# GmxMahdi/compute-raytracer

Measured on AMD Instinct MI355X. Metric: Mrays/s at 3840x2160, 1024 spheres, 8 bounces, higher is better.
Workload: dtype f32; 1 GPU; C3: 3840x2160, 1024 spheres (seed 358), 8 bounces, constant sky, reference default camera/light; mode=fast, variant=0, rays_per_frame=46143642, frames_in_flight=4, parallelism=row-tiles x1

## Files before the change

### compute_raytracer_amd/csrc/rt_bvh.hip

```cpp
#include <algorithm>
#include <cmath>
#include <cstdlib>
#include <vector>

#include "rt_filter.h"

#define RT_BVH_KAPPA 6.103515625e-05f
#define RT_BVH_REV_DELTA 0.0051f
#define RT_BVH_REV_DELTA_REL 7.62939453125e-06f
#define RT_BVH_REV_SLACK 2.44140625e-04f
#define RT_BVH_REV_SLACK_ABS 4.76837158203125e-07f

#ifndef RT_BVH_GRAB
#define RT_BVH_GRAB 256u
#endif
#ifndef RT_BVH_TAIL_SMALL
#define RT_BVH_TAIL_SMALL 16
#endif
#ifndef RT_BVH_TAIL_SERIAL
#define RT_BVH_TAIL_SERIAL 12
#endif
#ifndef RT_BVH_TAIL_LARGE
#define RT_BVH_TAIL_LARGE 28
#endif

namespace rtk {

__host__ __device__ inline uint32_t bvh_lds_l0(uint32_t n_nodes, uint32_t base) {
    uint32_t l0 = 1024u;
    const uint32_t need = (4u * (n_nodes + 1u) + 2u) / 3u;
    if (base + l0 < need) l0 = need - base;
    return (l0 + 15u) & ~15u;
}
__host__ __device__ inline uint32_t bvh_gap_waves(uint32_t n_nodes, uint32_t waves) {
    const uint32_t k = (bvh_lds_l0(n_nodes, 0u) - 1024u) / 512u;
    return k < waves ? k : waves;
}
__host__ __device__ constexpr uint32_t bvh_list_bytes(bool nlds, uint32_t cap) { return nlds ? 128u * (cap + 1u) : 256u * cap; }
__host__ __device__ inline uint32_t bvh_lds_lists(uint32_t n_nodes, uint32_t base) {
    const uint32_t l0 = bvh_lds_l0(n_nodes, base);
    return 4u * (base + l0) - base + 16u * ((n_nodes + 4u) & ~3u);
}

__global__ void bvh_fill_leaves(float4* rec, const uint32_t* link, uint32_t n_nodes, const float4* geo_f) {
    const uint32_t i = blockIdx.x * blockDim.x + threadIdx.x;
    if (i >= n_nodes) return;
    const uint32_t l = link[i];
    if (l & 0x80000000u) rec[i] = geo_f[l & 0x7FFFFFFFu];
}

__device__ __forceinline__ double wave_max_f64(double v) {
#pragma unroll
    for (int off = 32; off > 0; off >>= 1) v = fmax(v, __shfl_xor(v, off, 64));
    return v;
}
__device__ __forceinline__ double wave_min_f64(double v) {
#pragma unroll
    for (int off = 32; off > 0; off >>= 1) v = fmin(v, __shfl_xor(v, off, 64));
    return v;
}

__global__ __launch_bounds__(256) void bvh_refit(float4* __restrict__ rec, const uint32_t* __restrict__ link,
                                                  uint32_t n_nodes, const float* __restrict__ records) {
    const uint32_t node = blockIdx.x * 4u + (threadIdx.x >> 6), lane = threadIdx.x & 63u;
    if (node >= n_nodes) return;
    const uint32_t lk = link[node];
    if (lk & 0x80000000u) return;
    const uint32_t first = node + 1u, end = lk >> 2;
    auto sphere = [&](uint32_t j, double c[3], double& r) -> bool {
        if (j >= end) return false;
        const uint32_t l = link[j];
        if (!(l & 0x80000000u)) return false;
        const float* s = records + 8u * (size_t)(l & 0x7FFFFFFFu);
        for (int a = 0; a < 3; ++a) { const double v = (double)s[a]; c[a] = v == v ? v : 0.0; }
        const double rv = fabs((double)s[7]);
        r = rv == rv ? rv : 0.0;
        return true;
    };
    auto radius_at = [&](const double P[3], double far[3]) -> double {
        double best = -1.0, bc[3] = {0.0, 0.0, 0.0};
        for (uint32_t j = first + lane; j < end; j += 64u) {
            double c[3], r;
            if (!sphere(j, c, r)) continue;
            const double dx = c[0] - P[0], dy = c[1] - P[1], dz = c[2] - P[2];
            const double d = sqrt(dx * dx + dy * dy + dz * dz) + r;
            if (d > best) { best = d; bc[0] = c[0]; bc[1] = c[1]; bc[2] = c[2]; }
        }
        const double R = wave_max_f64(best);
        const uint64_t who = __ballot(best == R);
        const int src = who ? (int)__builtin_ctzll(who) : 0;
        for (int a = 0; a < 3; ++a) far[a] = __shfl(bc[a], src, 64);
        return R;
    };
    double mn[3] = {INFINITY, INFINITY, INFINITY}, mx[3] = {-INFINITY, -INFINITY, -INFINITY};
    for (uint32_t j = first + lane; j < end; j += 64u) {
        double c[3], r;
        if (!sphere(j, c, r)) continue;
        for (int a = 0; a < 3; ++a) { mn[a] = fmin(mn[a], c[a] - r); mx[a] = fmax(mx[a], c[a] + r); }
    }
    double P[3];
    for (int a = 0; a < 3; ++a) P[a] = 0.5 * (wave_min_f64(mn[a]) + wave_max_f64(mx[a]));
    double far[3];
    double Rp = radius_at(P, far);
    for (int it = 0; it < 32; ++it) {
        const double sx = far[0] - P[0], sy = far[1] - P[1], sz = far[2] - P[2];
        const double len = sqrt(sx * sx + sy * sy + sz * sz);
        if (!(len > 1e-12)) break;
        const double Q[3] = {P[0] + sx / len * 0.05 * Rp, P[1] + sy / len * 0.05 * Rp, P[2] + sz / len * 0.05 * Rp};
        double farq[3];
        const double Rq = radius_at(Q, farq);
        if (!(Rq < Rp)) break;
        P[0] = Q[0]; P[1] = Q[1]; P[2] = Q[2]; Rp = Rq;
        far[0] = farq[0]; far[1] = farq[1]; far[2] = farq[2];
    }
    const float C[3] = {(float)P[0], (float)P[1], (float)P[2]};
    const double Cd[3] = {(double)C[0], (double)C[1], (double)C[2]};
    double unused[3];
    double R = radius_at(Cd, unused);
    R *= RT_BVH_SIGMA;
    const double c2 = Cd[0] * Cd[0] + Cd[1] * Cd[1] + Cd[2] * Cd[2];
    const double k = c2 * (1.0 - (double)RT_FILTER_EPS) - R * R * (1.0 + (double)RT_FILTER_KAPPA);
    if (lane == 0)
        rec[node] = make_float4(C[0] * RT_FILTER_SCALE, C[1] * RT_FILTER_SCALE, C[2] * RT_FILTER_SCALE,
                                (float)(k * (double)RT_FILTER_SCALE2));
}

#ifdef RT_BVH_COUNT
#define g_steps steps_acc
__device__ unsigned long long g_wave_clock[3 * 8192];
#endif
__device__ __forceinline__ float min0(float b) {
    float d; asm("v_min_f32 %0, 0, %1" : "=v"(d) : "v"(b)); return d;
}

__device__ __forceinline__ void exact_any_order(v3 center, float r2, int s, v3 o, v3 d, float fa, float ta,
                                                float& nearest, int& idx) {
    const v3 oc = sub(o, center);
    const float b = 2.0f * dot(d, oc);
    const float c = dot(oc, oc) - r2;
    const float disc = b * b - fa * c;
    if (disc > 0.0f && b < 0.0f) {
        const float t = (-b - sqrtf(disc)) / ta;
        if (t > 0.001f && (t < nearest || (t == nearest && idx >= 0 && s < idx))) {
            nearest = t;
            idx = s;
        }
    }
}

__device__ __forceinline__ void reversed_shadow_walk(bool shadow, v3 L, float light_l1, v3 P, v3 s, v3& wo, v3& wd, float& madd) {
    const v3 dl = sub(P, L);
    const float l1 = (__builtin_fabsf(dl.x) + __builtin_fabsf(dl.y)) + __builtin_fabsf(dl.z);
    const float la = l1 + light_l1;
    const float delta = __builtin_fmaf(la, RT_BVH_REV_DELTA_REL, RT_BVH_REV_DELTA);
    const float lb = l1 + delta;
    const float slack = __builtin_fmaf(lb * lb, RT_BVH_REV_SLACK, (la * la) * RT_BVH_REV_SLACK_ABS);
    if (shadow) {
        wo = V(__builtin_fmaf(delta, s.x, P.x), __builtin_fmaf(delta, s.y, P.y), __builtin_fmaf(delta, s.z, P.z));
        wd = V(-s.x, -s.y, -s.z);
        madd = slack;
    }
}

template <bool SGN, bool NLDS, int CAP, bool ROOMY>
__device__ __forceinline__ void trace_bvh(const uint32_t tail, const float4* __restrict__ R, const uint32_t* __restrict__ L, uint32_t n,
                                          const float4* __restrict__ geo, uint32_t* slot, unsigned long long* best,
                                          uint32_t& i, v3 o, v3 d, v3 wo, v3 wd, float madd, float& nearest, int& idx
#ifdef RT_BVH_COUNT
                                          , uint32_t& steps_acc
#endif
                                          ) {
    const float a = dot(wd, wd);
    const float inv = __builtin_amdgcn_rsqf(a) * (1.0f + RT_BVH_KAPPA);
    const v3 h = V(wd.x * inv, wd.y * inv, wd.z * inv);
    const v3 os = V(wo.x * RT_FILTER_SCALE, wo.y * RT_FILTER_SCALE, wo.z * RT_FILTER_SCALE);
    const v3 m = V(-2.0f * os.x, -2.0f * os.y, -2.0f * os.z);
    const float p = dot(h, os);
    const float q = __builtin_fmaf(-madd, RT_FILTER_SCALE2, dot(os, os) * (1.0f - RT_FILTER_EPS));
    constexpr bool CLAMPED = SGN && NLDS;
    constexpr float kT = 2.168404344971009e-19f;
    constexpr float kT2 = 4.70197740328915e-38f;
    const v3 hs = V(h.x * kT, h.y * kT, h.z * kT);
    const v3 ms = V(m.x * kT2, m.y * kT2, m.z * kT2);
    const float ps = -p * kT, qs = q * kT2;
    typedef __attribute__((address_space(3))) uint32_t* lds_u32_w;
    typedef __attribute__((address_space(3))) uint16_t* lds_u16_w;
    const uint32_t wa0 = (uint32_t)(uintptr_t)slot;
    uint32_t wa = wa0;

    constexpr bool L16 = NLDS;
    typedef __attribute__((address_space(3))) const uint16_t* lds_u16;
    typedef __attribute__((address_space(3))) const uint32_t* lds_u32r;
    auto drain = [&]() {
        const uint32_t lane = threadIdx.x & 63u;
        const uint32_t cnt = L16 ? (wa - wa0) >> 7 : (wa - wa0) >> 8;
        uint32_t* const pool = slot - lane;
        const uint32_t top = wa0 - 2u * lane + 128u * (uint32_t)(CAP + 1);
        uint32_t total = 0;
        uint32_t lim = cnt;
        uint32_t again = 0;
        best[lane] = ((unsigned long long)__float_as_uint(nearest) << 32) | (unsigned long long)(uint32_t)idx;
      for (;;) {
        if (L16) {
            total = 0;
            uint32_t kstop = 0;
            bool stopped = false;
#pragma unroll
            for (int k = CAP - 1; k >= 0; --k) {
                const uint64_t m = __ballot((uint32_t)k < lim);
                if (m == 0ull) continue;
                const uint32_t need = (uint32_t)__popcll(m);
                if (!stopped && 4u * (total + need) > 128u * (uint32_t)(CAP + 1 - k)) { stopped = true; kstop = (uint32_t)k + 1u; }
                if (stopped) continue;
                uint32_t e = 0;
                if ((uint32_t)k < lim) e = *(lds_u16)(uintptr_t)(wa0 + 128u * (uint32_t)k);
                const uint32_t pos = total + __builtin_amdgcn_mbcnt_hi((uint32_t)(m >> 32), __builtin_amdgcn_mbcnt_lo((uint32_t)m, 0u));
                if ((uint32_t)k < lim) *(lds_u32_w)(uintptr_t)(top - 4u - 4u * pos) = (lane << 24) | e;
                total += need;
                asm volatile("" : "+s"(total));
            }
            again = stopped ? 1u : 0u;
            if (stopped) lim = lim < kstop ? lim : kstop;
        } else {
        for (uint32_t k = 0;; ++k) {
            const uint64_t m = __ballot(k < cnt);
            if (m == 0ull) break;
            uint32_t e = 0;
            if (k < cnt) e = slot[k * 64u];
            const uint32_t pos = total + (uint32_t)__popcll(m & ((1ull << lane) - 1ull));
            if (k < cnt) pool[pos] = (lane << 24) | (e & 0x00FFFFFFu);
            total += (uint32_t)__popcll(m);
        }
        }
        for (uint32_t i = lane; __ballot(i < total) != 0ull; i += 64u) {
#ifdef RT_BVH_COUNT
            if (RT_BVH_COUNT == 4) g_steps += lane == 0u ? 1u : 0u;
            if (RT_BVH_COUNT == 5) g_steps += i < total ? 1u : 0u;
#endif
            const uint32_t e = i < total ? (L16 ? *(lds_u32r)(uintptr_t)(top - 4u - 4u * i) : pool[i]) : (lane << 24);
            const int owner = (int)(e >> 24);
            const int si = (int)(e & 0x00FFFFFFu);
            typedef float f4r __attribute__((ext_vector_type(4)));
            f4r gr;
            asm volatile("global_load_dwordx4 %0, %1, %2" : "=&v"(gr) : "v"((uint32_t)si << 4), "s"(geo) : "memory");
            const v3 oo = V(__shfl(o.x, owner, 64), __shfl(o.y, owner, 64), __shfl(o.z, owner, 64));
            const v3 od = V(__shfl(d.x, owner, 64), __shfl(d.y, owner, 64), __shfl(d.z, owner, 64));
            if (i < total) {
                float a2 = dot(od, od);
                asm volatile("s_waitcnt vmcnt(0)" : "+v"(gr), "+v"(a2) : : "memory");
                const float4 g = make_float4(gr.x, gr.y, gr.z, gr.w);
                const v3 oc = sub(oo, V(g.x, g.y, g.z));
                const float b = 2.0f * dot(od, oc);
                const float c = dot(oc, oc) - g.w;
                const float disc = b * b - (4.0f * a2) * c;
                if (disc > 0.0f && b < 0.0f) {
                    const float t = (-b - sqrtf(disc)) / (2.0f * a2);
                    if (t > 0.001f && t < 9999.0f)
                        atomicMin(&best[owner], ((unsigned long long)__float_as_uint(t) << 32) | (unsigned long long)(uint32_t)si);
                }
            }
        }
        if (!L16 || __builtin_amdgcn_readfirstlane((int)again) == 0) break;
      }
        __builtin_amdgcn_fence(__ATOMIC_ACQ_REL, "wavefront");
        const unsigned long long r = best[lane];
        nearest = __uint_as_float((uint32_t)(r >> 32));
        idx = (int)(uint32_t)r;
        wa = wa0;
    };

    typedef __attribute__((address_space(3))) const uint32_t* lds_u32;
    typedef float f4v __attribute__((ext_vector_type(4)));
    typedef __attribute__((address_space(3))) const f4v* lds_f4;
    const uint32_t l0 = NLDS ? (uint32_t)(uintptr_t)L : 0u;
    auto fetch = [&](uint32_t j, float4& g, uint32_t& lk) {
        if (NLDS) {
            const f4v gv = *(lds_f4)(uintptr_t)j;
            lk = *(lds_u32)(uintptr_t)(j >> 2);
            g = make_float4(gv.x, gv.y, gv.z, gv.w);
        } else {
            lk = *reinterpret_cast<const uint32_t*>(reinterpret_cast<const char*>(L) + j);
            g = *reinterpret_cast<const float4*>(reinterpret_cast<const char*>(R) + 4u * (size_t)j);
        }
    };
    auto passes = [&](const float4& g) -> bool {
        if (CLAMPED) {
            float nb;
            const float part = fma_vvv(hs.y, g.y, fma_vvv(hs.x, g.x, ps));
            asm("v_fma_f32 %0, %1, %2, %3 clamp" : "=v"(nb) : "v"(hs.z), "v"(g.z), "v"(part));
            const float cp = fma_vvv(ms.z, g.z, fma_vvv(ms.y, g.y, fma_vvv(ms.x, g.x, g.w)));
            return __builtin_fmaf(nb, nb, -qs) > cp;
        } else {
            const float b = fnma_vvv(h.z, g.z, fnma_vvv(h.y, g.y, fnma_vvv(h.x, g.x, p)));
            const float cp = fma_vvv(m.z, g.z, fma_vvv(m.y, g.y, fma_vvv(m.x, g.x, g.w)));
            const float bm = SGN ? min0(b) : b;
            return __builtin_fmaf(bm, bm, -q) > cp;
        }
    };
    auto append = [&](uint32_t lk) {
        if (L16) {
            *(lds_u16_w)(uintptr_t)wa = (uint16_t)lk;
            asm("v_add_u32_e32 %0, 0x80, %0" : "+v"(wa));
        } else if (NLDS) {
            *(lds_u32_w)(uintptr_t)wa = lk;
            asm("v_add_u32_e32 %0, 0x100, %0" : "+v"(wa));
        } else {
            *(lds_u32_w)(uintptr_t)wa = lk;
            wa += 256u;
        }
    };
    const uint32_t jn = NLDS ? 4u * (4u * n + l0) : 4u * n;
    uint32_t j = NLDS ? 4u * (4u * i + l0) : 4u * i;
    const uint64_t walking0 = __ballot(j != jn);
    uint64_t walking = walking0;
    float4 g;
    uint32_t lk;
    fetch(j, g, lk);
    while (walking != 0ull) {
#ifdef RT_BVH_COUNT
        if (RT_BVH_COUNT == 1) g_steps += (threadIdx.x & 63u) == 0u ? 2u : 0u;
#endif
#pragma unroll
        for (int k = 0; k < 4; ++k) {
            const bool pass = passes(g);
            const bool leaf = (int)lk < 0;
#ifdef RT_BVH_COUNT
            if (RT_BVH_COUNT == 2) g_steps += j != jn ? 1u : 0u;
            if (RT_BVH_COUNT == 6) g_steps += leaf ? 1u : 0u;
            if (RT_BVH_COUNT == 7) g_steps += (!leaf && pass) ? 1u : 0u;
            if (RT_BVH_COUNT == 8) g_steps += (!leaf && lk != j) ? 1u : 0u;
#endif
            const uint32_t here = lk;
            j = (leaf || pass) ? j + (NLDS ? 16u : 4u) : lk;
            fetch(j, g, lk);
            if (leaf && pass) append(here);
        }
        if (__builtin_expect(__ballot(wa >= wa0 + (L16 ? 128u : 256u) * (uint32_t)(CAP - 3)) != 0ull, 0)) {
            drain();
            if (!ROOMY) fetch(j, g, lk);
        }
        walking = __ballot(j != jn);
        if (walking != walking0 && (uint32_t)__builtin_popcountll(walking) < tail) break;
    }
    drain();
    i = NLDS ? ((j >> 2) - l0) >> 2 : j >> 2;
}

inline bool lds_fits(size_t k, size_t bytes) { return k * ((bytes + 1279u) / 1280u) <= 128u; }
template <int WAVES, bool SGN, bool NLDS, int CAP, bool FLAT>
__global__ __launch_bounds__(64 * WAVES, WAVES == 16 ? 4 : 6) void bvh_pixels(const RtFrameArgs A) {
    extern __shared__ float4 lds[];
    const uint32_t n = A.bvh_nodes;
    const uint32_t n4 = (n + 4u) & ~3u;
    char* const lds_b = reinterpret_cast<char*>(lds);
    const uint32_t base = (uint32_t)(uintptr_t)lds;
    const uint32_t l0off = bvh_lds_l0(n, base);
    uint32_t* sL = reinterpret_cast<uint32_t*>(lds_b + (NLDS ? l0off : 0u));
    float4* sR = reinterpret_cast<float4*>(lds_b + (NLDS ? 4u * (base + l0off) - base : 0u));
    uint32_t* lists = reinterpret_cast<uint32_t*>(lds_b + (NLDS ? bvh_lds_lists(n, base) : 1024u));
    (void)n4;
    if (NLDS && base != 0u) { report_fault(A.rays, 1ull); return; }
    if (NLDS)
        for (uint32_t i = threadIdx.x; i <= n; i += 64 * WAVES) {
            float4 r = A.bvh_rec[i];
            if (SGN) r.w *= 4.70197740328915e-38f;
            sR[i] = r;
            const uint32_t lk = A.bvh_link[i];
            sL[i] = (int)lk < 0 ? lk : 4u * (lk + (uint32_t)(uintptr_t)sL);
        }
    const float4* R = NLDS ? sR : A.bvh_rec;
    const uint32_t* L = NLDS ? sL : A.bvh_link;
    const uint32_t lane = threadIdx.x & 63u;
    const uint32_t wave = (uint32_t)__builtin_amdgcn_readfirstlane((int)(threadIdx.x >> 6));
    constexpr uint32_t kListBytes = bvh_list_bytes(NLDS, (uint32_t)CAP);
    uint32_t* slot = reinterpret_cast<uint32_t*>(reinterpret_cast<char*>(lists) + wave * kListBytes + lane * (NLDS ? 2u : 4u));
    const uint32_t gapw = NLDS ? bvh_gap_waves(n, (uint32_t)WAVES) : 0u;
    unsigned long long* best = wave < gapw ? reinterpret_cast<unsigned long long*>(lds_b + 1024u) + wave * 64u
                                           : reinterpret_cast<unsigned long long*>(reinterpret_cast<char*>(lists) + WAVES * kListBytes) + (wave - gapw) * 64u;
    float* lut = reinterpret_cast<float*>(lds_b);
    for (uint32_t i = threadIdx.x; i < 256u; i += 64 * WAVES) lut[i] = (float)i / 255.0f;
    __syncthreads();

    const Scene sc = unpack_scene(A);
    v3 sky_c = V(0.0f, 0.0f, 0.0f);
    if (FLAT) {
        const v3 c = texel(A.face[0], 1, 1, 0, 0, lut);
        sky_c = V(__int_as_float(__builtin_amdgcn_readfirstlane(__float_as_int(c.x))),
                  __int_as_float(__builtin_amdgcn_readfirstlane(__float_as_int(c.y))),
                  __int_as_float(__builtin_amdgcn_readfirstlane(__float_as_int(c.z))));
    }
    auto flat_sky = [&](v3 r) -> v3 {
        const float z = (r.x * 0.0f + r.y * 0.0f) + r.z * 0.0f;
        return V(sky_c.x + z, sky_c.y + z, sky_c.z + z);
    };
    const float light_l1 = (__builtin_fabsf(sc.lightPos.x) + __builtin_fabsf(sc.lightPos.y)) + __builtin_fabsf(sc.lightPos.z);
    const uint32_t tiles_x = (A.W + 7u) / 8u;
    const uint32_t total = A.n_local_tiles * tiles_x * 64u;
    uint32_t cur = 0, end = 0;
    uint32_t chunk_ty = 0, chunk_tx = 0, chunk_first = ~0u;
    constexpr uint32_t kGrab = RT_BVH_GRAB;
    const uint32_t plenty = gridDim.x * (uint32_t)WAVES * 64u * 16u;
    uint32_t grab = 64u, trips = 0u;
    bool exhausted = false;
#ifdef RT_BVH_COUNT
    const uint64_t clk0 = wall_clock64();
    uint64_t clk_x = 0;
#endif

    bool active = false, shadow = false;
    uint32_t opix = 0, bounce = 0, nrays = 0;
    v3 ro = V(0, 0, 0), rd = V(0, 0, 1), color = V(1, 1, 1), fog = V(0, 0, 0);
    v3 normal = V(0, 0, 1), sdir = V(0, 0, 1), albedo = V(0, 0, 0);
    float dist = 0.0f, affect = 1.0f, sum = 0.0f, distance = 1.0f;
    uint32_t node = n;
    float t = 9999.0f;
    int idx = -1;

    for (;;) {
        ++trips;
        uint64_t idle = __ballot(!active);
        while (idle && !exhausted) {
            if (cur == end) {
                if (trips <= 2u && total - min(end, total) > plenty) grab = min(grab * 2u, kGrab);
                else if (trips > 8u) grab = 64u;
                trips = 0u;
                uint32_t base = 0;
#ifdef RT_BVH_COUNT
                const uint64_t clk_a = wall_clock64();
#endif
                if (lane == 0) base = atomicAdd(&A.qctrl[2], grab);
                base = __builtin_amdgcn_readfirstlane(base);
#ifdef RT_BVH_COUNT
                if (RT_BVH_COUNT == 14) nrays += lane == 0u ? 1u : 0u;
                if (RT_BVH_COUNT == 15) nrays += lane == 0u ? (uint32_t)(wall_clock64() - clk_a) : 0u;
#endif
                if (base >= total) {
                    exhausted = true;
#ifdef RT_BVH_COUNT
                    clk_x = wall_clock64();
#endif
                    break;
                }
                cur = base;
                end = min(base + grab, total);
            }
            if ((cur & 63u) == 0u || cur == chunk_first) {
                chunk_first = cur;
                chunk_ty = (cur >> 6) / tiles_x;
                chunk_tx = (cur >> 6) - chunk_ty * tiles_x;
            }
            const uint32_t tile_end = min(end, (cur & ~63u) + 64u);
            const uint32_t take = min((uint32_t)__popcll(idle), tile_end - cur);
            const uint32_t r = (uint32_t)__popcll(idle & ((1ull << lane) - 1ull));
            if (!active && r < take) {
                const uint32_t l = (cur + r) & 63u;
                const uint32_t ty = chunk_ty, tx = chunk_tx;
                const uint32_t x = tx * 8u + (l & 7u), row = l >> 3;
                const uint32_t y = (A.tile_first + ty * A.tile_step) * 8u + row;
                if (x < A.W && y < A.H) {
                    opix = (ty * 8u + row) * A.W + x;
                    ro = sc.cameraPos; rd = primary_dir(A, sc, x, y);
                    if (FLAT && sc.bounces == 0u) fog = scale(sc.minIntensity, flat_sky(rd));
                    color = V(1.0f, 1.0f, 1.0f); dist = 0.0f;
                    affect = 1.0f; sum = 0.0f; bounce = 0u;
                    shadow = false;
                    active = true;
                    node = 0u; t = 9999.0f; idx = -1;
                    if (sc.bounces == 0u) node = n;
                }
            }
            cur += take;
            idle = __ballot(!active);
        }
        if (__ballot(active) == 0ull) break;

        bool finished = active && sc.bounces == 0u;
        bool missed = false;
        const bool walking = node != n;
        v3 wo = ro, wd = shadow ? sdir : rd;
        float madd = 0.0f;
        if (SGN) reversed_shadow_walk(shadow, sc.lightPos, light_l1, ro, sdir, wo, wd, madd);
        else if (shadow) wo = sc.lightPos;
#ifdef RT_BVH_COUNT
        if (RT_BVH_COUNT == 3) nrays += lane == 0u ? 1u : 0u;
        trace_bvh<SGN, NLDS, CAP, WAVES == 16>(A.bvh_tail, R, L, n, A.geo, slot, best, node, shadow ? sc.lightPos : ro, shadow ? sdir : rd, wo, wd, madd, t, idx, nrays);
        if (walking && node == n) {
#else
        trace_bvh<SGN, NLDS, CAP, WAVES == 16>(A.bvh_tail, R, L, n, A.geo, slot, best, node, shadow ? sc.lightPos : ro, shadow ? sdir : rd, wo, wd, madd, t, idx);
        if (walking && node == n) {
            ++nrays;
#endif
            const float next = affect + sum;
            if (!shadow) {
                typedef float f3r __attribute__((ext_vector_type(3)));
                f3r hit_g, hit_c;
                {
                    const uint32_t off = (uint32_t)(idx < 0 ? 0 : idx) << 4;
                    asm volatile("global_load_dwordx3 %0, %2, %3\n\tglobal_load_dwordx3 %1, %2, %4"
                                 : "=&v"(hit_g), "=&v"(hit_c) : "v"(off), "s"(A.geo), "s"(A.col) : "memory");
                }
                if (bounce == 0u) dist = idx >= 0 ? t : 0.0f;
                v3 sky = V(0, 0, 0);
                if (FLAT && (bounce == 0u || idx < 0)) sky = scale(sc.minIntensity, flat_sky(rd));
                if (FLAT && bounce == 0u) fog = sky;
                if (idx < 0) {
                    if (FLAT) color = divs(add(scale(sum, color), scale(affect, sky)), next);
                    else missed = true;
                    finished = true;
                }
                asm volatile("s_waitcnt vmcnt(0)" : "+v"(hit_g), "+v"(hit_c) : : "memory");
                if (idx >= 0) {
                    albedo = V(hit_c.x, hit_c.y, hit_c.z);
                    const v3 pos = add(ro, scale(t, rd));
                    normal = normalize(sub(pos, V(hit_g.x, hit_g.y, hit_g.z)));
                    ro = pos;
                    rd = normalize(reflect(rd, normal));
                    sdir = normalize(sub(ro, sc.lightPos));
                    distance = length_of_unit(sdir);
                    shadow = true;
                    node = 0u; t = 9999.0f; idx = -1;
                }
            } else {
                const float intensity = light_term(sc, ro, normal, sdir, distance, idx >= 0, t);
                const v3 blended = scale(intensity, albedo);
                color = divs(add(scale(sum, color), scale(affect, blended)), next);
                affect = affect / 2.0f;
                sum = next;
                ++bounce;
                shadow = false;
                finished = bounce >= sc.bounces;
                if (!finished) { node = 0u; t = 9999.0f; idx = -1; }
            }
        }
        if (finished) {
            if (FLAT) {
                reinterpret_cast<uint32_t*>(A.out)[opix] = compose_pixel_sky(fog, color, dist);
            } else {
                A.fin[2u * opix] = make_float4(color.x, color.y, color.z, __uint_as_float(__float_as_uint(dist) | (missed ? 0x80000000u : 0u)));
                if (missed && bounce != 0u) A.fin[2u * opix + 1u] = make_float4(rd.x, rd.y, rd.z, __uint_as_float(bounce));
            }
            active = false;
        }
    }
#ifdef RT_BVH_COUNT
    if (RT_BVH_COUNT == 9) nrays = lane == 0u ? (uint32_t)(wall_clock64() - (clk_x ? clk_x : clk0)) : 0u;
    if (RT_BVH_COUNT == 10) nrays = lane == 0u ? (uint32_t)(wall_clock64() - clk0) : 0u;
    if (RT_BVH_COUNT == 13 && lane == 0u) {
        const uint32_t w = (blockIdx.x * WAVES + wave) % 8192u;
        g_wave_clock[3 * w] = clk0; g_wave_clock[3 * w + 1] = clk_x ? clk_x : clk0; g_wave_clock[3 * w + 2] = wall_clock64();
    }
#endif
    count_rays(A.rays, nrays);
}

__global__ __launch_bounds__(256) void sky_resolve(const RtFrameArgs A) {
    __shared__ float lut[256];
    lut[threadIdx.x] = (float)threadIdx.x / 255.0f;
    __syncthreads();
    const Scene sc = unpack_scene(A);
    const uint32_t slots = A.n_local_tiles * 8u * A.W;
    for (uint32_t opix = blockIdx.x * 256u + threadIdx.x; opix < slots; opix += gridDim.x * 256u) {
        const uint32_t lrow = opix / A.W, x = opix - lrow * A.W;
        const uint32_t y = (A.tile_first + (lrow >> 3) * A.tile_step) * 8u + (lrow & 7u);
        if (y >= A.H) continue;
        const float4 r0 = A.fin[2u * opix];
        const v3 fog = scale(sc.minIntensity, cube_sample<2>(A, primary_dir(A, sc, x, y), lut));
        v3 color = V(r0.x, r0.y, r0.z);
        const float dist = __uint_as_float(__float_as_uint(r0.w) & 0x7FFFFFFFu);
        if ((__float_as_uint(r0.w) >> 31) != 0u) {
            float4 r1 = make_float4(0.0f, 0.0f, 0.0f, 0.0f);
            if (dist != 0.0f) r1 = A.fin[2u * opix + 1u];
            const uint32_t k = min(__float_as_uint(r1.w), sc.bounces);
            float affect = 1.0f, sum = 0.0f;
            for (uint32_t i = 0; i < k; ++i) { const float next = affect + sum; affect = affect / 2.0f; sum = next; }
            const float next = affect + sum;
            const v3 sky = k == 0u ? fog : scale(sc.minIntensity, cube_sample<2>(A, V(r1.x, r1.y, r1.z), lut));
            color = divs(add(scale(sum, color), scale(affect, sky)), next);
        }
        reinterpret_cast<uint32_t*>(A.out)[opix] = compose_pixel_sky(fog, color, dist);
    }
}

template <int WAVES, bool SGN, bool NLDS, int CAP, int TAIL>
hipError_t launch_bvh_as(const RtFrameArgs& a0, size_t lds, hipStream_t s) {
    RtFrameArgs a = a0;
    a.bvh_tail = (uint32_t)TAIL;
    if (TAIL == RT_BVH_TAIL_SMALL && a.grid_share <= 1u) a.bvh_tail = RT_BVH_TAIL_SERIAL;
    else if (TAIL == RT_BVH_TAIL_SMALL && a.n_local_tiles * 8u * a.W < (1u << 22)) a.bvh_tail = 12u;
#ifdef RT_BVH_DEV_ENV
    if (const char* e = getenv("RT355_BVH_TAIL")) a.bvh_tail = (uint32_t)atoi(e);
#endif
    auto k = a.sky_flat ? bvh_pixels<WAVES, SGN, NLDS, CAP, true> : bvh_pixels<WAVES, SGN, NLDS, CAP, false>;
    if (lds > 48u * 1024u) {
        hipError_t e = hipFuncSetAttribute(reinterpret_cast<const void*>(k), hipFuncAttributeMaxDynamicSharedMemorySize, (int)lds);
        if (e != hipSuccess) return e;
    }
    uint32_t per_cu = WAVES == 8 ? 3u : (WAVES == 12 ? 2u : 1u);
    while (per_cu > 1u && !lds_fits(per_cu, lds)) --per_cu;
    const uint32_t pixels = a.n_local_tiles * ((a.W + 7u) / 8u) * 64u;
    uint32_t blocks = 256u * (per_cu ? per_cu : 1u);
    if (a.grid_share > 1u) blocks = WAVES == 8 ? std::max(256u, blocks / a.grid_share) : std::max(1u, blocks / a.grid_share);
    const uint32_t need = (pixels + 64u * WAVES - 1u) / (64u * WAVES);
    if (blocks > need) blocks = need;
#ifdef RT_BVH_DEV_ENV
    if (const char* e = getenv("RT355_BVH_BLOCKS")) if (atoi(e) > 0) blocks = std::min((uint32_t)atoi(e), need);
    if (const char* e = getenv("RT355_BVH_LDS_PAD")) {
        lds += (size_t)atoi(e);
        (void)hipFuncSetAttribute(reinterpret_cast<const void*>(k), hipFuncAttributeMaxDynamicSharedMemorySize, (int)lds);
    }
#endif
    if (!a.sky_flat && !a.fin) return hipErrorInvalidValue;
    g_rt_kernel_id = !NLDS ? RT_KID_HIERARCHY_GLOBAL : (WAVES == 8 ? RT_KID_HIERARCHY_8 : (WAVES == 12 ? RT_KID_HIERARCHY_12 : RT_KID_HIERARCHY_16));
    hipLaunchKernelGGL(k, dim3(blocks), dim3(64 * WAVES), lds, s, a);
    if (!a.sky_flat) return rt_launch_sky_resolve(a, s);
    return hipGetLastError();
}

template <bool SGN>
hipError_t launch_bvh(const RtFrameArgs& a, hipStream_t s) {
    if (a.n_local_tiles == 0 || a.W == 0) return hipSuccess;
    constexpr int CAP = 12;
    const size_t nodes = (size_t)bvh_lds_lists(a.bvh_nodes, 0u);
    const size_t cap = 160u * 1024u;
    auto room = [&](uint32_t waves, uint32_t entries) {
        return nodes + (size_t)waves * bvh_list_bytes(true, entries) + (size_t)(waves - bvh_gap_waves(a.bvh_nodes, waves)) * 512u;
    };
#ifdef RT_BVH_DEV_ENV
    if (const char* e = getenv("RT355_BVH_CAP")) {
        if (atoi(e) == 16 && lds_fits(3u, room(8u, 16u))) return launch_bvh_as<8, SGN, true, 16, RT_BVH_TAIL_SMALL>(a, room(8u, 16u), s);
        if (atoi(e) == 8 && lds_fits(3u, room(8u, 8u))) return launch_bvh_as<8, SGN, true, 8, RT_BVH_TAIL_SMALL>(a, room(8u, 8u), s);
        if (atoi(e) == 10 && lds_fits(3u, room(8u, 10u))) return launch_bvh_as<8, SGN, true, 10, RT_BVH_TAIL_SMALL>(a, room(8u, 10u), s);
    }
#endif
    if (lds_fits(3u, room(8u, CAP))) return launch_bvh_as<8, SGN, true, CAP, RT_BVH_TAIL_SMALL>(a, room(8u, CAP), s);
    if (lds_fits(2u, room(12u, CAP))) return launch_bvh_as<12, SGN, true, CAP, RT_BVH_TAIL_SMALL>(a, room(12u, CAP), s);
    if (lds_fits(2u, room(12u, 6u))) return launch_bvh_as<12, SGN, true, 6, RT_BVH_TAIL_SMALL>(a, room(12u, 6u), s);
#ifdef RT_BVH_DEV_ENV
    if (const char* e = getenv("RT355_BVH_CAP")) {
        if (atoi(e) == 16 && room(16u, 16u) <= cap) return launch_bvh_as<16, SGN, true, 16, RT_BVH_TAIL_LARGE>(a, room(16u, 16u), s);
        if (atoi(e) == 8 && room(16u, 8u) <= cap) return launch_bvh_as<16, SGN, true, 8, RT_BVH_TAIL_LARGE>(a, room(16u, 8u), s);
        if (atoi(e) == 6 && room(16u, 6u) <= cap) return launch_bvh_as<16, SGN, true, 6, RT_BVH_TAIL_LARGE>(a, room(16u, 6u), s);
    }
#endif
    if (room(16u, CAP) <= cap)     return launch_bvh_as<16, SGN, true, CAP, RT_BVH_TAIL_LARGE>(a, room(16u, CAP), s);
    if (room(16u, 6u) <= cap)      return launch_bvh_as<16, SGN, true, 6, RT_BVH_TAIL_LARGE>(a, room(16u, 6u), s);
    return launch_bvh_as<8, SGN, false, 8, RT_BVH_TAIL_LARGE>(a, 1024u + 8u * ((size_t)bvh_list_bytes(false, 8u) + 512u), s);
}

}

#ifdef RT_BVH_COUNT
extern "C" __attribute__((visibility("default"))) int rt_debug_wave_clock(unsigned long long* dst, size_t n) {
    return (int)hipMemcpyFromSymbol(dst, HIP_SYMBOL(rtk::g_wave_clock), n * sizeof(unsigned long long));
}
#endif

hipError_t rt_launch_sky_resolve(const RtFrameArgs& a, hipStream_t s) {
    const uint32_t slots = a.n_local_tiles * 8u * a.W;
    if (slots == 0u) return hipSuccess;
    hipLaunchKernelGGL(rtk::sky_resolve, dim3(std::min((slots + 255u) / 256u, 256u * 8u)), dim3(256), 0, s, a);
    return hipGetLastError();
}

hipError_t rt_launch_bvh(const RtFrameArgs& a, hipStream_t s) {
    return a.signed_filter ? rtk::launch_bvh<true>(a, s) : rtk::launch_bvh<false>(a, s);
}

hipError_t rt_launch_bvh_refit(float4* rec, const uint32_t* link, uint32_t n_nodes, const float* records, hipStream_t s) {
    if (n_nodes == 0) return hipSuccess;
    hipLaunchKernelGGL(rtk::bvh_refit, dim3((n_nodes + 3u) / 4u), dim3(256), 0, s, rec, link, n_nodes, records);
    return hipGetLastError();
}

hipError_t rt_launch_bvh_fill(float4* rec, const uint32_t* link, uint32_t n_nodes, const float4* geo_f, hipStream_t s) {
    if (n_nodes == 0) return hipSuccess;
    hipLaunchKernelGGL(rtk::bvh_fill_leaves, dim3((n_nodes + 255u) / 256u), dim3(256), 0, s, rec, link, n_nodes, geo_f);
    return hipGetLastError();
}
```

### compute_raytracer_amd/csrc/rt_device.h

```cpp
#pragma once
#include "rt_types.h"

namespace rtk {

struct v3 { float x, y, z; };
__device__ __forceinline__ v3 V(float x, float y, float z) { v3 r = {x, y, z}; return r; }
__device__ __forceinline__ v3 add(v3 a, v3 b) { return V(a.x + b.x, a.y + b.y, a.z + b.z); }
__device__ __forceinline__ v3 sub(v3 a, v3 b) { return V(a.x - b.x, a.y - b.y, a.z - b.z); }
__device__ __forceinline__ v3 scale(float s, v3 a) { return V(s * a.x, s * a.y, s * a.z); }
__device__ __forceinline__ v3 divs(v3 a, float s) { return V(a.x / s, a.y / s, a.z / s); }
__device__ __forceinline__ float dot(v3 a, v3 b) { return (a.x * b.x + a.y * b.y) + a.z * b.z; }
__device__ __forceinline__ float length(v3 a) { return sqrtf(dot(a, a)); }
__device__ __forceinline__ v3 normalize(v3 a) { return divs(a, length(a)); }
__device__ __forceinline__ float length_of_unit(v3 a) {
    const float x = dot(a, a);
    const int k = __float_as_int(x) - 0x3F800000;
    const float quick = __int_as_float(0x3F800000 + (k >> 1));
    const bool near_one = (uint32_t)(k + 4096) <= 8192u;
    if (__builtin_expect(__ballot(!near_one) == 0ull, 1)) return quick;
    return near_one ? quick : sqrtf(x);
}
__device__ __forceinline__ float clampf(float x, float lo, float hi) { return fminf(fmaxf(x, lo), hi); }
__device__ __forceinline__ v3 reflect(v3 e1, v3 e2) { return sub(e1, scale(2.0f * dot(e2, e1), e2)); }

__device__ __forceinline__ v3 texel(const uint8_t* __restrict__ f, int w, int h, int x, int y, const float* lut = nullptr) {
    x = x < 0 ? 0 : (x > w - 1 ? w - 1 : x);
    y = y < 0 ? 0 : (y > h - 1 ? h - 1 : y);
    const uchar4 p = *reinterpret_cast<const uchar4*>(f + 4u * ((size_t)y * (size_t)w + (size_t)x));
    if (lut) return V(lut[p.x], lut[p.y], lut[p.z]);
    return V((float)p.x / 255.0f, (float)p.y / 255.0f, (float)p.z / 255.0f);
}
__device__ __forceinline__ v3 lerp3(v3 a, v3 b, float f) { return add(a, scale(f, sub(b, a))); }

__device__ inline void cube_fold(int face, int i, int j, int n, int& nf, int& ni, int& nj) {
    const int S = 2 * i + 1 - n, T = 2 * j + 1 - n, m = n - 1;
    int x, y, z;
    if (face == 0)      { x = n;  y = -T; z = -S; }
    else if (face == 1) { x = -n; y = -T; z = S;  }
    else if (face == 2) { x = S;  y = n;  z = T;  }
    else if (face == 3) { x = S;  y = -n; z = -T; }
    else if (face == 4) { x = S;  y = -T; z = n;  }
    else                { x = -S; y = -T; z = -n; }
    const int major = face >> 1;
    const bool ox = major != 0 && (x > m || x < -m);
    const bool oy = major != 1 && (y > m || y < -m);
    if (major == 0) x = x > 0 ? m : -m;
    else if (major == 1) y = y > 0 ? m : -m;
    else z = z > 0 ? m : -m;
    int S2, T2;
    if (ox)      { nf = x > 0 ? 0 : 1; S2 = x > 0 ? -z : z; T2 = -y; }
    else if (oy) { nf = y > 0 ? 2 : 3; S2 = x; T2 = y > 0 ? z : -z; }
    else         { nf = z > 0 ? 4 : 5; S2 = z > 0 ? x : -x; T2 = -y; }
    ni = (S2 + m) >> 1;
    nj = (T2 + m) >> 1;
}

template <bool INDEXED = false>
__device__ __forceinline__ v3 cube_texel_at(const RtFrameArgs& A, int face, int n, int x, int y, const float* lut) {
    const uint8_t* f = INDEXED ? A.face[face] : A.face[0];
#pragma unroll
    for (int i = 1; i < 6; ++i)
        if (!INDEXED && face == i) f = A.face[i];
    const uchar4 p = *reinterpret_cast<const uchar4*>(f + 4u * ((size_t)y * (size_t)n + (size_t)x));
    if (lut) return V(lut[p.x], lut[p.y], lut[p.z]);
    return V((float)p.x / 255.0f, (float)p.y / 255.0f, (float)p.z / 255.0f);
}

template <bool INDEXED = false>
__device__ inline v3 cube_tap(const RtFrameArgs& A, int face, int n, int i, int j, const float* lut) {
    const bool oi = i < 0 || i >= n, oj = j < 0 || j >= n;
    if (!oi && !oj) return cube_texel_at<INDEXED>(A, face, n, i, j, lut);
    const int ci = i < 0 ? 0 : (i >= n ? n - 1 : i), cj = j < 0 ? 0 : (j >= n ? n - 1 : j);
    int f2, i2, j2;
    if (oi && oj) {
        const v3 a = cube_texel_at<INDEXED>(A, face, n, ci, cj, lut);
        cube_fold(face, i, cj, n, f2, i2, j2);
        const v3 b = cube_texel_at<INDEXED>(A, f2, n, i2, j2, lut);
        cube_fold(face, ci, j, n, f2, i2, j2);
        const v3 c = cube_texel_at<INDEXED>(A, f2, n, i2, j2, lut);
        return add(a, divs(add(sub(b, a), sub(c, a)), 3.0f));
    }
    cube_fold(face, i, j, n, f2, i2, j2);
    return cube_texel_at<INDEXED>(A, f2, n, i2, j2, lut);
}

template <int SKY = 0, bool INDEXED = false>
__device__ inline v3 cube_sample(const RtFrameArgs& A, v3 r, const float* lut = nullptr) {
    if (SKY == 1) {
        const float ax = fabsf(r.x), ay = fabsf(r.y), az = fabsf(r.z);
        float sc, tc, ma;
        if (az >= ax && az >= ay) { sc = r.x; tc = r.y; ma = az; }
        else if (ay >= ax)        { sc = r.x; tc = r.z; ma = ay; }
        else                      { sc = r.z; tc = r.y; ma = ax; }
        const v3 c = texel(A.face[0], 1, 1, 0, 0, lut);
        const float z = (sc / ma) * 0.0f + (tc / ma) * 0.0f;
        return V(c.x + z, c.y + z, c.z + z);
    }
    const float ax = fabsf(r.x), ay = fabsf(r.y), az = fabsf(r.z);
    int face; float sc, tc, ma;
    if (az >= ax && az >= ay) {
        if (r.z >= 0.0f) { face = 4; sc = r.x;  tc = -r.y; } else { face = 5; sc = -r.x; tc = -r.y; }
        ma = az;
    } else if (ay >= ax) {
        if (r.y >= 0.0f) { face = 2; sc = r.x; tc = r.z; } else { face = 3; sc = r.x; tc = -r.z; }
        ma = ay;
    } else {
        if (r.x >= 0.0f) { face = 0; sc = -r.z; tc = -r.y; } else { face = 1; sc = r.z; tc = -r.y; }
        ma = ax;
    }
    const uint8_t* f = INDEXED ? A.face[face] : A.face[0];
    int w = (int)(INDEXED ? A.fw[face] : A.fw[0]), h = (int)(INDEXED ? A.fh[face] : A.fh[0]);
#pragma unroll
    for (int i = 1; i < 6; ++i)
        if (!INDEXED && face == i) { f = A.face[i]; w = (int)A.fw[i]; h = (int)A.fh[i]; }
    const float s = 0.5f * (sc / ma) + 0.5f;
    const float t = 0.5f * (tc / ma) + 0.5f;
    const float u = s * (float)w - 0.5f;
    const float v = t * (float)h - 0.5f;
    const float fu = floorf(u), fv = floorf(v);
    const float wu = u - fu, wv = v - fv;
    const int x0 = (int)fu, y0 = (int)fv;
    if (SKY == 1 || (SKY == 0 && A.sky_flat)) {
        const v3 c = texel(f, 1, 1, 0, 0, lut);
        const float z = wu * 0.0f + wv * 0.0f;
        return V(c.x + z, c.y + z, c.z + z);
    }
    if (SKY == 1) return V(0, 0, 0);
    if (A.sky_seamless && x0 >= 0 && x0 + 1 < w && y0 >= 0 && y0 + 1 < w) {
        uint2 r0, r1;
        __builtin_memcpy(&r0, f + 4u * ((size_t)y0 * (size_t)w + (size_t)x0), 8);
        __builtin_memcpy(&r1, f + 4u * ((size_t)(y0 + 1) * (size_t)w + (size_t)x0), 8);
        auto un = [&](uint32_t p) {
            if (lut) return V(lut[p & 255u], lut[(p >> 8) & 255u], lut[(p >> 16) & 255u]);
            return V((float)(p & 255u) / 255.0f, (float)((p >> 8) & 255u) / 255.0f, (float)((p >> 16) & 255u) / 255.0f);
        };
        return lerp3(lerp3(un(r0.x), un(r0.y), wu), lerp3(un(r1.x), un(r1.y), wu), wv);
    }
    if (A.sky_seamless && x0 >= -1 && x0 < w && y0 >= -1 && y0 < w) {
        v3 top = V(0, 0, 0), row = V(0, 0, 0);
#pragma unroll 1
        for (int k = 0; k < 2; ++k) {
            top = row;
            const v3 a = cube_tap<INDEXED>(A, face, w, x0, y0 + k, lut), b = cube_tap<INDEXED>(A, face, w, x0 + 1, y0 + k, lut);
            row = lerp3(a, b, wu);
        }
        return lerp3(top, row, wv);
    }
    const v3 c00 = texel(f, w, h, x0, y0, lut), c10 = texel(f, w, h, x0 + 1, y0, lut);
    const v3 c01 = texel(f, w, h, x0, y0 + 1, lut), c11 = texel(f, w, h, x0 + 1, y0 + 1, lut);
    return lerp3(lerp3(c00, c10, wu), lerp3(c01, c11, wu), wv);
}

__device__ __forceinline__ uint32_t unorm8(float c) {
    if (!(c == c)) return 0u;
    c = clampf(c, 0.0f, 1.0f);
    return (uint32_t)floorf(c * 255.0f + 0.5f);
}

struct Scene {
    v3 cameraPos, forwards, right, up, lightPos;
    float lightIntensity, minIntensity;
    uint32_t bounces;
};
__device__ __forceinline__ Scene unpack_scene(const RtFrameArgs& A) {
    Scene s;
    s.cameraPos = V(A.p[0], A.p[1], A.p[2]);
    s.forwards = V(A.p[4], A.p[5], A.p[6]);
    s.right = V(A.p[8], A.p[9], A.p[10]);
    s.up = V(A.p[12], A.p[13], A.p[14]);
    s.lightPos = V(A.p[16], A.p[17], A.p[18]);
    s.lightIntensity = A.p[19];
    s.minIntensity = A.p[20];
    const float mb = A.p[21];
    s.bounces = 0;
    if (mb > 0.0f) s.bounces = mb >= 4294967040.0f ? 4294967295u : (uint32_t)mb;
    return s;
}

__device__ __forceinline__ v3 primary_dir(const RtFrameArgs& A, const Scene& sc, uint32_t x, uint32_t y) {
    const float hc = ((float)(int)x - (float)A.W / 2.0f) / (float)A.W * 2.0f;
    const float vc = ((float)A.H / 2.0f - (float)(int)y) / (float)A.W * 2.0f;
    return normalize(add(add(sc.forwards, scale(hc, sc.right)), scale(vc, sc.up)));
}

__device__ __forceinline__ uint32_t compose_pixel_sky(v3 sky, v3 color, float dist) {
    const float k = clampf((30.0f - dist) / 30.0f, 0.0f, 1.0f);
    const v3 px = add(scale(k, color), scale(1.0f - k, sky));
    return unorm8(px.x) | (unorm8(px.y) << 8) | (unorm8(px.z) << 16) | 0xFF000000u;
}
__device__ __forceinline__ uint32_t compose_pixel(const RtFrameArgs& A, const Scene& sc, v3 dir0, v3 color, float dist) {
    return compose_pixel_sky(scale(sc.minIntensity, cube_sample(A, dir0)), color, dist);
}

__device__ __forceinline__ float light_term(const Scene& sc, v3 dest, v3 normal, v3 sdir, float distance,
                                            bool shit, float st) {
    if (shit) {
        const v3 hp = add(sc.lightPos, scale(st, sdir));
        const v3 dv = sub(hp, dest);
        if (dot(dv, dv) < 0x1.a36e2cp-16f) {
            const float power = clampf(dot(normal, V(-sdir.x, -sdir.y, -sdir.z)), sc.minIntensity, 1.0f);
            const float cap = sc.lightIntensity / (sc.lightIntensity + distance);
            return power * cap;
        }
    }
    return sc.minIntensity;
}

__device__ __forceinline__ uint32_t wave_sum(uint32_t v) {
#pragma unroll
    for (int off = 32; off > 0; off >>= 1) v += __shfl_xor(v, off, 64);
    return v;
}

__device__ __forceinline__ void report_fault(unsigned long long* counter, unsigned long long code) {
    if (threadIdx.x == 0) atomicMax(counter + 1, code);
}

__device__ __forceinline__ void count_wave_rays(unsigned long long* counter, uint32_t wave_rays) {
    const uint32_t wave_id = (blockIdx.y * gridDim.x + blockIdx.x) * (blockDim.x >> 6) + (threadIdx.x >> 6);
    atomicAdd(counter + (size_t)(wave_id % RT_RAY_COUNTERS) * (RT_RAY_COUNTER_STRIDE / 8u), (unsigned long long)wave_rays);
}

__device__ __forceinline__ void count_rays(unsigned long long* counter, uint32_t nrays) {
    const uint32_t wave_id = (blockIdx.y * gridDim.x + blockIdx.x) * (blockDim.x >> 6) + (threadIdx.x >> 6);
    unsigned long long* part = counter + (size_t)(wave_id % RT_RAY_COUNTERS) * (RT_RAY_COUNTER_STRIDE / 8u);
    const uint64_t live = __ballot(1);
    if (live == ~0ull) {
        const uint32_t tot = wave_sum(nrays);
        if ((threadIdx.x & 63u) == 0) atomicAdd(part, (unsigned long long)tot);
    } else {
        atomicAdd(part, (unsigned long long)nrays);
    }
}

}
```

Before: 31200 Mrays/s.

## Restructure bounce shading so divergent lanes share divisions and normalizations

```diff
diff --git a/compute_raytracer_amd/csrc/rt_bvh.hip b/compute_raytracer_amd/csrc/rt_bvh.hip
--- a/compute_raytracer_amd/csrc/rt_bvh.hip
+++ b/compute_raytracer_amd/csrc/rt_bvh.hip
@@ -346,6 +346,15 @@
     i = NLDS ? ((j >> 2) - l0) >> 2 : j >> 2;
 }
 
+template <bool ROOT>
+__device__ __forceinline__ v3 shared_div(bool root, v3 a, v3 d) {
+    if (ROOT) {
+        const float l = length(a);
+        if (root) d = V(l, l, l);
+    }
+    return V(a.x / d.x, a.y / d.y, a.z / d.z);
+}
+
 inline bool lds_fits(size_t k, size_t bytes) { return k * ((bytes + 1279u) / 1280u) <= 128u; }
 template <int WAVES, bool SGN, bool NLDS, int CAP, bool FLAT>
 __global__ __launch_bounds__(64 * WAVES, WAVES == 16 ? 4 : 6) void bvh_pixels(const RtFrameArgs A) {
@@ -393,7 +402,8 @@
         const float z = (r.x * 0.0f + r.y * 0.0f) + r.z * 0.0f;
         return V(sky_c.x + z, sky_c.y + z, sky_c.z + z);
     };
-    const float light_l1 = (__builtin_fabsf(sc.lightPos.x) + __builtin_fabsf(sc.lightPos.y)) + __builtin_fabsf(sc.lightPos.z);
+    const float light_l1 = __int_as_float(__builtin_amdgcn_readfirstlane(__float_as_int(
+        (__builtin_fabsf(sc.lightPos.x) + __builtin_fabsf(sc.lightPos.y)) + __builtin_fabsf(sc.lightPos.z))));
     const uint32_t tiles_x = (A.W + 7u) / 8u;
     const uint32_t total = A.n_local_tiles * tiles_x * 64u;
     uint32_t cur = 0, end = 0;
@@ -408,6 +418,7 @@
 #endif
 
     bool active = false, shadow = false;
+    bool done = false;
     uint32_t opix = 0, bounce = 0, nrays = 0;
     v3 ro = V(0, 0, 0), rd = V(0, 0, 1), color = V(1, 1, 1), fog = V(0, 0, 0);
     v3 normal = V(0, 0, 1), sdir = V(0, 0, 1), albedo = V(0, 0, 0);
@@ -417,8 +428,70 @@
     int idx = -1;
 
     for (;;) {
+        const bool refl = done && !shadow, shd = done && shadow;
+        const bool hit = refl && idx >= 0;
+        bool finished = active && sc.bounces == 0u;
+        bool missed = false;
+        const float next = affect + sum;
+        v3 a1 = V(sc.lightIntensity, 0.0f, 0.0f), d1 = V(sc.lightIntensity + distance, next, next);
+        if (refl) {
+            typedef float f3r __attribute__((ext_vector_type(3)));
+            f3r hit_g, hit_c;
+            {
+                const uint32_t off = (uint32_t)(idx < 0 ? 0 : idx) << 4;
+                asm volatile("global_load_dwordx3 %0, %2, %3\n\tglobal_load_dwordx3 %1, %2, %4"
+                             : "=&v"(hit_g), "=&v"(hit_c) : "v"(off), "s"(A.geo), "s"(A.col) : "memory");
+            }
+            if (bounce == 0u) dist = idx >= 0 ? t : 0.0f;
+            v3 sky = V(0, 0, 0);
+            if (FLAT && (bounce == 0u || idx < 0)) sky = scale(sc.minIntensity, flat_sky(rd));
+            if (FLAT && bounce == 0u) fog = sky;
+            if (idx < 0) {
+                if (FLAT) { a1 = add(scale(sum, color), scale(affect, sky)); d1 = V(next, next, next); }
+                else missed = true;
+                finished = true;
+            }
+            asm volatile("s_waitcnt vmcnt(0)" : "+v"(hit_g), "+v"(hit_c) : : "memory");
+            if (idx >= 0) {
+                albedo = V(hit_c.x, hit_c.y, hit_c.z);
+                const v3 pos = add(ro, scale(t, rd));
+                a1 = sub(pos, V(hit_g.x, hit_g.y, hit_g.z));
+                ro = pos;
+            }
+        }
+        const v3 q1 = shared_div<true>(hit, a1, d1);
+        if (hit) normal = q1;
+        if (FLAT && refl && !hit) color = q1;
+        v3 a2 = sub(ro, sc.lightPos);
+        if (shd) {
+            float power = 0.0f;
+            const bool lit = light_lit(sc, ro, normal, sdir, idx >= 0, t, power);
+            const float intensity = lit ? power * q1.x : sc.minIntensity;
+            const v3 blended = scale(intensity, albedo);
+            a2 = add(scale(sum, color), scale(affect, blended));
+        }
+        const v3 q2 = shared_div<true>(hit, a2, V(next, next, next));
+        if (hit) {
+            rd = reflect(rd, normal);
+            sdir = q2;
+            distance = length_of_unit(sdir);
+            shadow = true;
+            node = 0u; t = 9999.0f; idx = -1;
+        }
+        if (shd) {
+            color = q2;
+            affect = affect / 2.0f;
+            sum = next;
+            ++bounce;
+            shadow = false;
+            finished = bounce >= sc.bounces;
+            if (!finished) { node = 0u; t = 9999.0f; idx = -1; }
+        }
+
         ++trips;
-        uint64_t idle = __ballot(!active);
+        bool fresh = false;
+        uint32_t npix = 0, nx = 0, ny = 0;
+        uint64_t idle = __ballot(!active || finished);
         while (idle && !exhausted) {
             if (cur == end) {
                 if (trips <= 2u && total - min(end, total) > plenty) grab = min(grab * 2u, kGrab);
@@ -451,31 +524,47 @@
             }
             const uint32_t tile_end = min(end, (cur & ~63u) + 64u);
             const uint32_t take = min((uint32_t)__popcll(idle), tile_end - cur);
-            const uint32_t r = (uint32_t)__popcll(idle & ((1ull << lane) - 1ull));
-            if (!active && r < take) {
+            const uint32_t r = __builtin_amdgcn_mbcnt_hi((uint32_t)(idle >> 32), __builtin_amdgcn_mbcnt_lo((uint32_t)idle, 0u));
+            if ((!active || finished) && !fresh && r < take) {
                 const uint32_t l = (cur + r) & 63u;
                 const uint32_t ty = chunk_ty, tx = chunk_tx;
                 const uint32_t x = tx * 8u + (l & 7u), row = l >> 3;
                 const uint32_t y = (A.tile_first + ty * A.tile_step) * 8u + row;
                 if (x < A.W && y < A.H) {
-                    opix = (ty * 8u + row) * A.W + x;
-                    ro = sc.cameraPos; rd = primary_dir(A, sc, x, y);
-                    if (FLAT && sc.bounces == 0u) fog = scale(sc.minIntensity, flat_sky(rd));
-                    color = V(1.0f, 1.0f, 1.0f); dist = 0.0f;
-                    affect = 1.0f; sum = 0.0f; bounce = 0u;
-                    shadow = false;
-                    active = true;
-                    node = 0u; t = 9999.0f; idx = -1;
-                    if (sc.bounces == 0u) node = n;
+                    npix = (ty * 8u + row) * A.W + x;
+                    nx = x; ny = y;
+                    fresh = true;
                 }
             }
             cur += take;
-            idle = __ballot(!active);
-        }
+            idle = __ballot((!active || finished) && !fresh);
+        }
+        const v3 q3 = shared_div<false>(false, V(primary_hnum(A, nx), primary_vnum(A, ny), 30.0f - dist),
+                                        V((float)A.W, (float)A.W, 30.0f));
+        if (finished) {
+            if (FLAT) {
+                reinterpret_cast<uint32_t*>(A.out)[opix] = compose_pixel_fq(fog, color, q3.z);
+            } else {
+                A.fin[2u * opix] = make_float4(color.x, color.y, color.z, __uint_as_float(__float_as_uint(dist) | (missed ? 0x80000000u : 0u)));
+                if (missed && bounce != 0u) A.fin[2u * opix + 1u] = make_float4(rd.x, rd.y, rd.z, __uint_as_float(bounce));
+            }
+            active = false;
+        }
+        if (fresh) {
+            opix = npix;
+            ro = sc.cameraPos; rd = primary_unnormalised(sc, q3.x, q3.y);
+            color = V(1.0f, 1.0f, 1.0f); dist = 0.0f;
+            affect = 1.0f; sum = 0.0f; bounce = 0u;
+            shadow = false;
+            active = true;
+            node = 0u; t = 9999.0f; idx = -1;
+            if (sc.bounces == 0u) node = n;
+        }
+        const v3 q4 = normalize(rd);
+        if (hit || fresh) rd = q4;
+        if (FLAT && fresh && sc.bounces == 0u) fog = scale(sc.minIntensity, flat_sky(rd));
         if (__ballot(active) == 0ull) break;
 
-        bool finished = active && sc.bounces == 0u;
-        bool missed = false;
         const bool walking = node != n;
         v3 wo = ro, wd = shadow ? sdir : rd;
         float madd = 0.0f;
@@ -484,63 +573,12 @@
 #ifdef RT_BVH_COUNT
         if (RT_BVH_COUNT == 3) nrays += lane == 0u ? 1u : 0u;
         trace_bvh<SGN, NLDS, CAP, WAVES == 16>(A.bvh_tail, R, L, n, A.geo, slot, best, node, shadow ? sc.lightPos : ro, shadow ? sdir : rd, wo, wd, madd, t, idx, nrays);
-        if (walking && node == n) {
+        done = walking && node == n;
 #else
         trace_bvh<SGN, NLDS, CAP, WAVES == 16>(A.bvh_tail, R, L, n, A.geo, slot, best, node, shadow ? sc.lightPos : ro, shadow ? sdir : rd, wo, wd, madd, t, idx);
-        if (walking && node == n) {
-            ++nrays;
-#endif
-            const float next = affect + sum;
-            if (!shadow) {
-                typedef float f3r __attribute__((ext_vector_type(3)));
-                f3r hit_g, hit_c;
-                {
-                    const uint32_t off = (uint32_t)(idx < 0 ? 0 : idx) << 4;
-                    asm volatile("global_load_dwordx3 %0, %2, %3\n\tglobal_load_dwordx3 %1, %2, %4"
-                                 : "=&v"(hit_g), "=&v"(hit_c) : "v"(off), "s"(A.geo), "s"(A.col) : "memory");
-                }
-                if (bounce == 0u) dist = idx >= 0 ? t : 0.0f;
-                v3 sky = V(0, 0, 0);
-                if (FLAT && (bounce == 0u || idx < 0)) sky = scale(sc.minIntensity, flat_sky(rd));
-                if (FLAT && bounce == 0u) fog = sky;
-                if (idx < 0) {
-                    if (FLAT) color = divs(add(scale(sum, color), scale(affect, sky)), next);
-                    else missed = true;
-                    finished = true;
-                }
-                asm volatile("s_waitcnt vmcnt(0)" : "+v"(hit_g), "+v"(hit_c) : : "memory");
-                if (idx >= 0) {
-                    albedo = V(hit_c.x, hit_c.y, hit_c.z);
-                    const v3 pos = add(ro, scale(t, rd));
-                    normal = normalize(sub(pos, V(hit_g.x, hit_g.y, hit_g.z)));
-                    ro = pos;
-                    rd = normalize(reflect(rd, normal));
-                    sdir = normalize(sub(ro, sc.lightPos));
-                    distance = length_of_unit(sdir);
-                    shadow = true;
-                    node = 0u; t = 9999.0f; idx = -1;
-                }
-            } else {
-                const float intensity = light_term(sc, ro, normal, sdir, distance, idx >= 0, t);
-                const v3 blended = scale(intensity, albedo);
-                color = divs(add(scale(sum, color), scale(affect, blended)), next);
-                affect = affect / 2.0f;
-                sum = next;
-                ++bounce;
-                shadow = false;
-                finished = bounce >= sc.bounces;
-                if (!finished) { node = 0u; t = 9999.0f; idx = -1; }
-            }
-        }
-        if (finished) {
-            if (FLAT) {
-                reinterpret_cast<uint32_t*>(A.out)[opix] = compose_pixel_sky(fog, color, dist);
-            } else {
-                A.fin[2u * opix] = make_float4(color.x, color.y, color.z, __uint_as_float(__float_as_uint(dist) | (missed ? 0x80000000u : 0u)));
-                if (missed && bounce != 0u) A.fin[2u * opix + 1u] = make_float4(rd.x, rd.y, rd.z, __uint_as_float(bounce));
-            }
-            active = false;
-        }
+        done = walking && node == n;
+        if (done) ++nrays;
+#endif
     }
 #ifdef RT_BVH_COUNT
     if (RT_BVH_COUNT == 9) nrays = lane == 0u ? (uint32_t)(wall_clock64() - (clk_x ? clk_x : clk0)) : 0u;
@@ -550,7 +588,7 @@
         g_wave_clock[3 * w] = clk0; g_wave_clock[3 * w + 1] = clk_x ? clk_x : clk0; g_wave_clock[3 * w + 2] = wall_clock64();
     }
 #endif
-    count_rays(A.rays, nrays);
+    count_rays_wave(A.rays, nrays, wave);
 }
 
 __global__ __launch_bounds__(256) void sky_resolve(const RtFrameArgs A) {
diff --git a/compute_raytracer_amd/csrc/rt_device.h b/compute_raytracer_amd/csrc/rt_device.h
--- a/compute_raytracer_amd/csrc/rt_device.h
+++ b/compute_raytracer_amd/csrc/rt_device.h
@@ -206,6 +206,29 @@
     return sc.minIntensity;
 }
 
+__device__ __forceinline__ float primary_hnum(const RtFrameArgs& A, uint32_t x) { return (float)(int)x - (float)A.W / 2.0f; }
+__device__ __forceinline__ float primary_vnum(const RtFrameArgs& A, uint32_t y) { return (float)A.H / 2.0f - (float)(int)y; }
+__device__ __forceinline__ v3 primary_unnormalised(const Scene& sc, float hq, float vq) {
+    const float hc = hq * 2.0f, vc = vq * 2.0f;
+    return add(add(sc.forwards, scale(hc, sc.right)), scale(vc, sc.up));
+}
+__device__ __forceinline__ bool light_lit(const Scene& sc, v3 dest, v3 normal, v3 sdir, bool shit, float st, float& power) {
+    if (shit) {
+        const v3 hp = add(sc.lightPos, scale(st, sdir));
+        const v3 dv = sub(hp, dest);
+        if (dot(dv, dv) < 0x1.a36e2cp-16f) {
+            power = clampf(dot(normal, V(-sdir.x, -sdir.y, -sdir.z)), sc.minIntensity, 1.0f);
+            return true;
+        }
+    }
+    return false;
+}
+__device__ __forceinline__ uint32_t compose_pixel_fq(v3 sky, v3 color, float fq) {
+    const float k = clampf(fq, 0.0f, 1.0f);
+    const v3 px = add(scale(k, color), scale(1.0f - k, sky));
+    return unorm8(px.x) | (unorm8(px.y) << 8) | (unorm8(px.z) << 16) | 0xFF000000u;
+}
+
 __device__ __forceinline__ uint32_t wave_sum(uint32_t v) {
 #pragma unroll
     for (int off = 32; off > 0; off >>= 1) v += __shfl_xor(v, off, 64);
@@ -219,6 +242,18 @@
 __device__ __forceinline__ void count_wave_rays(unsigned long long* counter, uint32_t wave_rays) {
     const uint32_t wave_id = (blockIdx.y * gridDim.x + blockIdx.x) * (blockDim.x >> 6) + (threadIdx.x >> 6);
     atomicAdd(counter + (size_t)(wave_id % RT_RAY_COUNTERS) * (RT_RAY_COUNTER_STRIDE / 8u), (unsigned long long)wave_rays);
+}
+
+__device__ __forceinline__ void count_rays_wave(unsigned long long* counter, uint32_t nrays, uint32_t wave_in_block) {
+    const uint32_t wave_id = (blockIdx.y * gridDim.x + blockIdx.x) * (blockDim.x >> 6) + wave_in_block;
+    unsigned long long* part = counter + (size_t)(wave_id % RT_RAY_COUNTERS) * (RT_RAY_COUNTER_STRIDE / 8u);
+    const uint64_t live = __ballot(1);
+    if (live == ~0ull) {
+        const uint32_t tot = wave_sum(nrays);
+        if ((threadIdx.x & 63u) == 0) atomicAdd(part, (unsigned long long)tot);
+    } else {
+        atomicAdd(part, (unsigned long long)nrays);
+    }
 }
 
 __device__ __forceinline__ void count_rays(unsigned long long* counter, uint32_t nrays) {
```

Measured after the change: 33050 Mrays/s, median of 6. 1.06x the previous value.
